# matthewygf/Tiresias

Hardware: AMD Instinct MI355X
Metric: avg JCT + makespan on NSDI'19 Microsoft trace, 8×MI355X cluster (lower is better)
Workload: dtype bf16

## Files before the change

### csrc/bindings/ops.cpp

```cpp
#include <array>
#include <ATen/ATen.h>
#include <c10/hip/HIPStream.h>
#include <torch/library.h>

#include <functional>
#include <map>
#include <mutex>
#include <sstream>
#include <tuple>
#include <vector>

#include "tam/kernels.h"
#include "tam/launch.h"
#include "tam/gemm8p.h"

using at::Tensor;
using c10::optional;

namespace {

hipStream_t cur_stream(const Tensor& t) {
  return c10::hip::getCurrentHIPStream(t.device().index()).stream();
}

// ... 831 lines not shown
void maxpool_backward_op(const Tensor& dy, const Tensor& idx, const Tensor& dx, int64_t R, int64_t S,
                         int64_t st, int64_t pad) {
  check_bf16(dy, "dy"); check_bf16(dx, "dx");
  tam::maxpool_backward(bp(dy), idx.data_ptr<uint8_t>(), bpm(dx), (int)dx.size(0), (int)dx.size(1),
                        (int)dx.size(2), (int)dx.size(3), (int)dy.size(1), (int)dy.size(2), (int)R,
                        (int)S, (int)st, (int)pad, cur_stream(dy));
}
void avgpool_forward_op(const Tensor& x, const Tensor& y) {
  check_bf16(x, "x"); check_bf16(y, "y"); check_contig(x, "x");
  tam::avgpool_forward(bp(x), bpm(y), (int)x.size(0), (int)(x.size(1) * x.size(2)), (int)x.size(3),
                       cur_stream(x));
}
void avgpool_backward_op(const Tensor& dy, const Tensor& dx) {
  check_bf16(dy, "dy"); check_bf16(dx, "dx"); check_contig(dx, "dx");
  tam::avgpool_backward(bp(dy), bpm(dx), (int)dx.size(0), (int)(dx.size(1) * dx.size(2)),
                        (int)dx.size(3), cur_stream(dy));
}

void softmax_xent_op(const Tensor& logits, const Tensor& labels, const optional<Tensor>& dlogits,
                     const Tensor& loss_rows, double smoothing, double grad_scale,
                     int64_t ignore_index, int64_t tm_b) {
  check_bf16(logits, "logits"); check_contig(logits, "logits");
  TORCH_CHECK(labels.scalar_type() == at::kLong && labels.is_cuda() && labels.is_contiguous(),
              "tam.xent: labels contiguous int64 GPU");
  check_f32(loss_rows, "loss_rows");
  const int64_t V = logits.size(-1), rows = logits.numel() / V;
  TORCH_CHECK(labels.numel() == rows && loss_rows.numel() == rows, "tam.xent: row count");
  TORCH_CHECK(tm_b <= 0 || rows % tm_b == 0, "tam.xent: tm_b must divide the rows");
  tam::softmax_xent(bp(logits), labels.data_ptr<int64_t>(), opt_ptr<tam::bf16_t>(dlogits),
                    loss_rows.data_ptr<float>(), rows, (int)V, (float)smoothing, (float)grad_scale,
                    ignore_index, cur_stream(logits), tm_b);
}

void embedding_forward_op(const Tensor& table, const Tensor& ids, const Tensor& out, double scale, int64_t tm_b,
                          const optional<Tensor>& pos) {
  check_bf16(table, "table"); check_bf16(out, "out"); check_contig(table, "table");
  TORCH_CHECK(ids.scalar_type() == at::kLong && ids.is_contiguous(), "tam.embedding: ids");
  const int64_t D = table.size(1);
  TORCH_CHECK(D % 8 == 0, "tam.embedding: D % 8");
  TORCH_CHECK(out.numel() == ids.numel() * D, "tam.embedding: out size");
  TORCH_CHECK(tm_b <= 0 || ids.numel() % tm_b == 0, "tam.embedding: tm_b must divide the ids");
  const tam::bf16_t* pp = nullptr;
  int64_t prow = 0;
  if (pos.has_value() && pos->defined()) {
    check_bf16(*pos, "pos"); check_contig(*pos, "pos");
    TORCH_CHECK(pos->dim() == 2 && pos->size(1) == D, "tam.embedding: pos must be [S][D]");
    prow = pos->size(0);
    TORCH_CHECK(prow > 0 && (tm_b > 0 ? ids.numel() / tm_b == prow : ids.numel() % prow == 0),
                "tam.embedding: pos rows must equal the sequence length");
    pp = bp(*pos);
  }
  tam::embedding_forward(bp(table), ids.data_ptr<int64_t>(), bpm(out), ids.numel(), (int)D,
                         (float)scale, cur_stream(table), table.size(0), tm_b, pp, prow);
}
void embedding_backward_op(const Tensor& dout, const Tensor& ids, const Tensor& gtable, double scale, int64_t tm_b) {
  check_bf16(dout, "dout"); check_f32(gtable, "gtable"); check_contig(dout, "dout");
  TORCH_CHECK(ids.scalar_type() == at::kLong && ids.is_contiguous() && gtable.dim() == 2 &&
                  dout.numel() == ids.numel() * gtable.size(1), "tam.embedding_backward: shapes");
  TORCH_CHECK(tm_b <= 0 || ids.numel() % tm_b == 0, "tam.embedding_backward: tm_b must divide the ids");
  tam::embedding_backward(bp(dout), ids.data_ptr<int64_t>(), gtable.data_ptr<float>(), ids.numel(),
                          (int)gtable.size(1), (float)scale, cur_stream(dout), gtable.size(0), tm_b);
}

void conv_dma_policy_op(int64_t p) { tam::conv_dma_policy((int)p); }
void conv_halo_policy_op(int64_t p) { tam::conv_halo_policy((int)p); }
void colsum_policy_op(int64_t p) { tam::colsum_policy((int)p); }
void attn_short_policy_op(int64_t p) { tam::attn_short_policy((int)p); }
void conv_wgrad_c64_policy_op(int64_t p) { tam::conv_wgrad_c64_policy((int)p); }
void conv_wgrad_order_op(int64_t p) { tam::conv_wgrad_order((int)p); }
void conv_stem_policy_op(int64_t p) { tam::conv_stem_policy((int)p); }
void conv_wgrad_slab_policy_op(int64_t p) { tam::conv_wgrad_slab_policy((int)p); }
void conv_wgrad_force_op(int64_t bm, int64_t bn, int64_t splits, int64_t noatomic) {
  tam::conv_wgrad_force((int)bm, (int)bn, (int)splits, (int)noatomic);
}
int g_dma_policy = 1;
TAM_KNOB(g_dma_policy)
void gemm_dma_policy_op(int64_t p, int64_t cfg) {
  g_dma_policy = (int)p;
  tam::gemm_dma_policy(p == 2 ? 1 : 0, (int)cfg);
}

void gemm8p_policy_op(int64_t mode, int64_t tile) { tam::gemm8p_policy((int)mode, (int)tile); }
void gemm_pw_policy_op(int64_t on) { tam::gemm_pw_policy((int)on); }

std::string policy_names_op() {
  std::string out;
  for (const auto& k : tam::knob_registry()) {
    if (!out.empty()) out += ",";
    out += k.name;
  }
  return out;
}
std::vector<int64_t> policy_state_op() {
  std::vector<int64_t> v;
  for (const auto& k : tam::knob_registry()) v.push_back(*k.p);
  return v;
}
void policy_load_op(std::vector<int64_t> v) {
  auto& reg = tam::knob_registry();
  TORCH_CHECK(v.size() == reg.size(), "policy_load: ", v.size(), " values for ", reg.size(), " knobs");
  for (size_t i = 0; i < reg.size(); ++i) *reg[i].p = (int)v[i];
}
void gemm8p_group_op(int64_t g) { tam::gemm8p_group((int)g); }
void gemm8p_slab_force_op(int64_t sp) { tam::gemm8p_slab_force((int)sp); }
void gemm8p_sk_force_op(int64_t on) { g_sk_force = on != 0; }
void conv_split_policy_op(int64_t p) { tam::conv_split_policy((int)p); }
void optim_grid_op(int64_t b) { tam::optim_grid((int)b); }
void optim_variant_op(int64_t v) { tam::optim_variant((int)v); }
void gemm_skinny_policy_op(int64_t on, int64_t sp, int64_t nst) {
  tam::gemm_skinny_policy((int)on, (int)sp, (int)nst);
}

void gemm_force_op(int64_t cfg, int64_t splits) {
  tam::gemm_force((int)cfg, (int)splits);
  g_forced = cfg >= 0 || splits >= 1;
}

void colsum_op(const Tensor& x, const Tensor& out) {
  check_bf16(x, "x"); check_f32(out, "out"); check_contig(x, "x");
  const int64_t C = x.size(-1);
  Tensor ws = at::empty({C % 8 == 0 ? (int64_t)tam::COLSUM_MAX_BLOCKS * C : 1},
                        x.options().dtype(at::kFloat));
  tam::colsum(bp(x), out.data_ptr<float>(), ws.data_ptr<float>(), x.numel() / C, (int)C,
              cur_stream(x));
}
void relu_backward_op(const Tensor& dy, const Tensor& y, const Tensor& dx) {
  check_bf16(dy, "dy"); check_bf16(y, "y"); check_bf16(dx, "dx");
  tam::relu_backward(bp(dy), bp(y), bpm(dx), dy.numel(), cur_stream(dy));
}
void sum_scale_op(const Tensor& x, const Tensor& out, double scale) {
  check_f32(x, "x"); check_f32(out, "out"); check_contig(x, "x");
  TORCH_CHECK(out.numel() >= 1, "tam.sum_scale: out");
  tam::sum_scale(x.data_ptr<float>(), x.numel(), out.data_ptr<float>(), (float)scale, cur_stream(x));
}
static std::pair<int64_t, int64_t> row_view(const Tensor& t, const char* what) {
  TORCH_CHECK(t.is_cuda() && t.scalar_type() == at::kBFloat16 && t.dim() >= 1 && t.stride(-1) == 1,
              "tam.rows_sum: ", what, " must be a bf16 CUDA tensor with unit last stride");
  const int64_t C = t.size(-1);
  int64_t ld = t.dim() >= 2 ? t.stride(-2) : C;
  for (int64_t d = t.dim() - 2; d >= 1; --d)
    TORCH_CHECK(t.size(d) == 1 || t.size(d - 1) == 1 || t.stride(d - 1) == t.stride(d) * t.size(d),
                "tam.rows_sum: ", what, " leading dims do not collapse to one row pitch");
  TORCH_CHECK(C % 8 == 0 && ld % 8 == 0 && (((uintptr_t)t.data_ptr()) & 15) == 0,
              "tam.rows_sum: ", what, " needs C % 8 == 0 and 16-B aligned rows");
  return {C, ld};
}
void rows_sum_op(at::TensorList outs, at::TensorList ins, at::IntArrayRef n_in) {
  TORCH_CHECK(!outs.empty() && outs.size() <= 4 && outs.size() == n_in.size(), "tam.rows_sum: 1-4 jobs");
  const int64_t R = outs[0].numel() / outs[0].size(-1);
  tam::RowJobs jb{};
  size_t q = 0;
  for (size_t j = 0; j < outs.size(); ++j) {
    auto [C, ld] = row_view(outs[j], "out");
    TORCH_CHECK(outs[j].numel() / C == R, "tam.rows_sum: every job needs the same row count");
    TORCH_CHECK(n_in[j] >= 1 && n_in[j] <= 4 && q + n_in[j] <= ins.size(), "tam.rows_sum: n_in");
    tam::RowJob& r = jb.job[j];
    r.out = bpm(outs[j]); r.ld_out = ld; r.C = (int)C; r.n_in = (int)n_in[j];
    for (int k = 0; k < r.n_in; ++k, ++q) {
      auto [Ci, ldi] = row_view(ins[q], "in");
      TORCH_CHECK(Ci == C && ins[q].numel() / Ci == R, "tam.rows_sum: input shape");
      r.in[k] = bp(ins[q]); r.ld_in[k] = ldi;
    }
  }
  TORCH_CHECK(q == ins.size(), "tam.rows_sum: unused inputs");
  tam::rows_sum(jb, (int)outs.size(), R, cur_stream(outs[0]));
}
// ... 206 lines not shown
                               act.data_ptr<float>(), (int)T, (int)B, (int)Hd, reverse ? 1 : 0,
                               (unsigned*)sp, cur_stream(gx), pl_opts(job_err, grids, rsv, zeroed));
}
bool lstm_seq_bwd_op(const Tensor& act, const Tensor& cs, const Tensor& dH, const Tensor& w_hh,
                     const Tensor& dG, bool reverse, const Tensor& sync, const optional<Tensor>& job_err,
                     int64_t grids, int64_t rsv, bool zeroed) {
  check_f32(act, "act"); check_f32(cs, "cs"); check_bf16(w_hh, "w_hh");
  TORCH_CHECK(dH.is_cuda() && (dH.scalar_type() == at::kFloat || dH.scalar_type() == at::kBFloat16),
              "tam.lstm_seq_backward: dH must be an f32 or bf16 CUDA tensor");
  const int dh_bf16 = dH.scalar_type() == at::kBFloat16 ? 1 : 0;
  check_bf16(dG, "dG");
  TORCH_CHECK(cs.dim() == 3 && cs.is_contiguous(), "tam.lstm_seq_backward: cs [T][B][Hd]");
  const int64_t T = cs.size(0), B = cs.size(1), Hd = cs.size(2);
  check_sync(sync, B);
  TORCH_CHECK(w_hh.is_contiguous() && w_hh.size(0) == 4 * Hd && w_hh.size(1) == Hd,
              "tam.lstm_seq_backward: w_hh [4Hd][Hd]");
  TORCH_CHECK(dH.dim() == 3 && dH.size(0) == T && dH.size(1) == B && dH.size(2) == Hd && dH.stride(2) == 1 &&
                  dH.stride(1) >= Hd && dH.stride(0) == B * dH.stride(1),
              "tam.lstm_seq_backward: dH [T][B][Hd] with unit column stride and uniform row pitch");
  TORCH_CHECK(act.is_contiguous() && act.numel() == T * B * 5 * Hd && dG.is_contiguous() &&
                  dG.numel() == T * B * 4 * Hd,
              "tam.lstm_seq_backward: act / dG shapes");
  int* sp = sync.data_ptr<int>();
  return tam::lstm_seq_backward(act.data_ptr<float>(), cs.data_ptr<float>(), (const float*)dH.data_ptr(),
                                bp(w_hh), bpm(dG), (int)T, (int)B, (int)Hd, reverse ? 1 : 0, (unsigned*)sp,
                                dh_bf16, (int)dH.stride(1), cur_stream(act), pl_opts(job_err, grids, rsv, zeroed));
}

void lstm_seq_policy_op(int64_t ch) { tam::lstm_seq_policy((int)ch); }
void lstm_seq_shards_op(int64_t ns) { tam::lstm_seq_shards((int)ns); }
void lstm_seq_residency_op(int64_t grids, int64_t rsv) { tam::lstm_seq_residency((int)grids, (int)rsv); }
int64_t lstm_persist_timeouts_op(bool reset) { return tam::lstm_persist_timeouts(reset); }
void lstm_seq_spin_limit_op(int64_t polls) { tam::lstm_seq_spin_limit(polls); }

void lstm_bwd_op(const Tensor& act, const optional<Tensor>& c_prev, const optional<Tensor>& dh,
                 const optional<Tensor>& dc_next, const optional<Tensor>& dgates,
                 const optional<Tensor>& dc_prev, const optional<Tensor>& dgates_bf16) {
  check_f32(act, "act");
  const int B = (int)act.size(0), Hd = (int)(act.size(1) / 5);
  tam::lstm_cell_backward(act.data_ptr<float>(), opt_ptr<const float>(c_prev), nullptr,
                          opt_ptr<const float>(dh), opt_ptr<const float>(dc_next),
                          opt_ptr<float>(dgates), opt_ptr<float>(dc_prev),
                          opt_ptr<tam::bf16_t>(dgates_bf16), B, Hd, c10::hip::getCurrentHIPStream(act.device().index()).stream());
}

}

TORCH_LIBRARY(tam, m) {
  m.def("gemm(Tensor a, bool a_kmajor, Tensor b, bool b_kmajor, Tensor(a!) c, int mode, Tensor? bias, bool relu, Tensor? mask, float alpha, bool allow_split, Tensor(b!)? colsum=None) -> ()", &gemm_op);
  m.def("conv_fwd(Tensor x, Tensor w, Tensor(a!) y, int stride, int pad, int dil, Tensor? bias, bool relu, Tensor(b!)? stats=None) -> int", &conv_fwd_op);
  m.def("conv_dgrad(Tensor dy, Tensor w, Tensor(a!) wt, Tensor(b!) dx, int stride, int pad, int dil, Tensor? mask) -> ()", &conv_dgrad_op);
  m.def("conv_weight_t_batch(Tensor[] w, Tensor(a!)[] wt) -> ()", &conv_weight_t_batch_op);
  m.def("gemm_wgrad_grouped(Tensor[] dy, Tensor[] x, Tensor(a!)[] dw, Tensor(b!)[] db, int[]? modes=None) -> ()", &gemm_wgrad_grouped_op);
  m.def("gemm_wgrad_grouped_ok(int M, int N, int K) -> bool", &gemm_wgrad_grouped_ok_op);
  m.def("gemm_grouped_tile(int tile) -> ()", &gemm_grouped_tile_op);
  m.def("conv_dgrad_pre(Tensor dy, Tensor w, Tensor wt, Tensor(a!) dx, int stride, int pad, int dil, Tensor? mask, Tensor(b!)? stats=None, Tensor? bnx=None, Tensor? bnmean=None, Tensor? bnrstd=None) -> int", &conv_dgrad_pre_op);
  m.def("conv_wgrad(Tensor dy, Tensor x, Tensor(a!) dw, int stride, int pad, int dil, int mode, Tensor(b!)? dbias=None, bool patch=True) -> ()", &conv_wgrad_op);
  m.def("conv_wgrad_deferred(Tensor dy, Tensor x, Tensor(a!) dw, int stride, int pad, int dil, int mode, Tensor(b!)? dbias, bool patch) -> (Tensor, int)", &conv_wgrad_deferred_op);
  m.def("wgrad_slab_reduce_many(Tensor[] slabs, int[] sp, Tensor(a!)[] dw, int[] mode) -> ()", &wgrad_slab_reduce_many_op);
  m.def("bn_forward(Tensor x, Tensor? res, Tensor(a!) y, Tensor gamma, Tensor beta, Tensor(b!)? run_mean, Tensor(c!)? run_var, Tensor(d!) save_mean, Tensor(e!) save_rstd, float eps, float momentum, bool relu, Tensor(f!)? sums=None, bool sums_ready=False, Tensor(g!)? ymask=None) -> ()", &bn_forward_op);
  m.def("bn_backward(Tensor dy, Tensor? y, Tensor x, Tensor mean, Tensor rstd, Tensor gamma, Tensor(a!) dx, Tensor(b!)? dres, Tensor(c!)? dgamma, Tensor(d!)? dbeta, bool relu, Tensor? addend=None, Tensor(e!)? sums=None, bool sums_ready=False, Tensor? ymask=None) -> ()", &bn_backward_op);
  m.def("ln_forward(Tensor x, Tensor g, Tensor b, Tensor(a!) y, Tensor(b!) mean, Tensor(c!) rstd, float eps, Tensor? addend=None, Tensor(d!)? sum_out=None, Tensor? drop_rec=None, int drop_site=0, int drop_thr=0, float drop_scale=1.0) -> ()", &ln_forward_op);
  m.def("ln_backward(Tensor dy, Tensor x, Tensor g, Tensor mean, Tensor rstd, Tensor(a!) dx, Tensor(b!) dg, Tensor(c!) db, Tensor? addend=None, Tensor(d!)? dr=None, Tensor? drop_rec=None, int drop_site=0, int drop_thr=0, float drop_scale=1.0) -> ()", &ln_backward_op);
  m.def("ln_backward_split(Tensor dy, Tensor x, Tensor g, Tensor mean, Tensor rstd, Tensor(a!) dx, Tensor(b!) ws, Tensor? addend=None, Tensor(c!)? dr=None, Tensor? drop_rec=None, int drop_site=0, int drop_thr=0, float drop_scale=1.0) -> int", &ln_backward_split_op);
  m.def("dropout_apply(Tensor x, Tensor(a!) y, Tensor rec, int site, int thr, float scale) -> ()", &dropout_apply_op);
  m.def("dropout_advance(Tensor(a!) rec) -> ()", &dropout_advance_op);
  m.def("col_reduce_acc(Tensor part, int nblk, int W, Tensor(a!) out0, Tensor(b!) out1, int split) -> ()", &col_reduce_acc_op);
  m.def("col_reduce_acc_batch(Tensor[] parts, int[] nblk, Tensor(a!)[] out0, Tensor(b!)[] out1) -> ()", &col_reduce_acc_batch_op);
  m.def("maxpool_forward(Tensor x, Tensor(a!) y, Tensor(b!) idx, int R, int S, int stride, int pad) -> ()", &maxpool_forward_op);
  m.def("maxpool_backward(Tensor dy, Tensor idx, Tensor(a!) dx, int R, int S, int stride, int pad) -> ()", &maxpool_backward_op);
  m.def("maxpool_k3s2_policy(int policy) -> ()", &maxpool_k3s2_policy_op);
  m.def("avgpool_forward(Tensor x, Tensor(a!) y) -> ()", &avgpool_forward_op);
  m.def("avgpool_backward(Tensor dy, Tensor(a!) dx) -> ()", &avgpool_backward_op);
  m.def("softmax_xent(Tensor logits, Tensor labels, Tensor(a!)? dlogits, Tensor(b!) loss_rows, float smoothing, float grad_scale, int ignore_index, int tm_b=0) -> ()", &softmax_xent_op);
  m.def("embedding_forward(Tensor table, Tensor ids, Tensor(a!) out, float scale, int tm_b=0, Tensor? pos=None) -> ()", &embedding_forward_op);
  m.def("embedding_backward(Tensor dout, Tensor ids, Tensor(a!) gtable, float scale, int tm_b=0) -> ()", &embedding_backward_op);
  m.def("sum_scale(Tensor x, Tensor(a!) out, float scale) -> ()", &sum_scale_op);
  m.def("rows_sum(Tensor[] outs, Tensor[] ins, int[] n_in) -> ()", &rows_sum_op);
  m.def("zero_(Tensor(a!) t) -> ()", &zero_op);
  m.def("colsum(Tensor x, Tensor(a!) out) -> ()", &colsum_op);
  m.def("gemm_force(int cfg, int splits) -> ()", &gemm_force_op);
  m.def("gemm8p_policy(int mode, int tile) -> ()", &gemm8p_policy_op);
  m.def("gemm_pw_policy(int on) -> ()", &gemm_pw_policy_op);
  m.def("policy_names() -> str", &policy_names_op);
  m.def("policy_state() -> int[]", &policy_state_op);
  m.def("policy_load(int[] v) -> ()", &policy_load_op);
  m.def("gemm8p_group(int g) -> ()", &gemm8p_group_op);
  m.def("gemm8p_slab_force(int sp) -> ()", &gemm8p_slab_force_op);
  m.def("gemm_skinny_policy(int on, int force_splits, int nst) -> ()", &gemm_skinny_policy_op);
  m.def("gemm8p_sk_force(int on) -> ()", &gemm8p_sk_force_op);
  m.def("conv_split_policy(int p) -> ()", &conv_split_policy_op);
  m.def("optim_variant(int v) -> ()", &optim_variant_op);
  m.def("optim_grid(int blocks) -> ()", &optim_grid_op);
  m.def("gemm_lib_policy(int policy) -> ()", &gemm_lib_policy_op);
  m.def("conv_dma_policy(int policy) -> ()", &conv_dma_policy_op);
  m.def("conv_wgrad_force(int bm, int bn, int splits, int noatomic=0) -> ()", &conv_wgrad_force_op);
  m.def("conv_wgrad_c64_policy(int policy) -> ()", &conv_wgrad_c64_policy_op);
  m.def("conv_wgrad_order(int flat) -> ()", &conv_wgrad_order_op);
  m.def("conv_stem_policy(int policy) -> ()", &conv_stem_policy_op);
  m.def("conv_wgrad_slab_policy(int policy) -> ()", &conv_wgrad_slab_policy_op);
  m.def("conv_halo_policy(int policy) -> ()", &conv_halo_policy_op);
  m.def("colsum_policy(int policy) -> ()", &colsum_policy_op);
  m.def("attn_short_policy(int policy) -> ()", &attn_short_policy_op);
  m.def("gemm_dma_policy(int policy, int cfg) -> ()", &gemm_dma_policy_op);
  m.def("gemm_routes() -> str", &gemm_routes_op);
  m.def("relu_backward(Tensor dy, Tensor y, Tensor(a!) dx) -> ()", &relu_backward_op);
  m.def("add(Tensor a, Tensor b, Tensor(a!) y) -> ()", &add_op);
  m.def("cast_f32_bf16(Tensor x, Tensor(a!) y) -> ()", &cast_op);
  m.def("sgd_step(Tensor(a!) w, Tensor(b!) g, Tensor(c!) mom, Tensor(d!) wb, float lr, float momentum, float wd, float gscale, bool nesterov, bool zero_grad, Tensor? guard=None, int zero_from=0, int wd_until=-1, Tensor? clip=None) -> ()", &sgd_op);
  m.def("adam_step(Tensor(a!) w, Tensor(b!) g, Tensor(c!) m, Tensor(d!) v, Tensor(e!) wb, float lr, float b1, float b2, float eps, float wd, int step, float gscale, bool zero_grad, Tensor? guard=None, int zero_from=0, int wd_until=-1, Tensor? clip=None) -> ()", &adam_op);
  m.def("grad_sumsq(Tensor g, Tensor(a!) partials) -> ()", &grad_sumsq_op);
  m.def("grad_clip_finalize(Tensor partials, float max_norm, float gscale, Tensor(a!) clip) -> ()", &grad_clip_finalize_op);
  m.def("grad_sumsq_blocks(int n) -> int", &grad_sumsq_blocks_op);
  m.def("lstm_guard_step(Tensor(a!) err) -> ()", &lstm_guard_step_op);
  m.def("attn_forward(Tensor q, Tensor k, Tensor v, Tensor(a!) o, Tensor(b!) lse, bool causal, float scale, Tensor? kv_len, Tensor? drop_rec=None, int drop_site=0, int drop_thr=0, float drop_scale=1.0) -> ()", &attn_forward_op);
  m.def("attn_backward(Tensor q, Tensor k, Tensor v, Tensor o, Tensor dout, Tensor lse, Tensor(a!) dq, Tensor(b!) dk, Tensor(c!) dv, Tensor(d!) dq_acc, Tensor(e!) delta, bool causal, float scale, Tensor? kv_len, Tensor? drop_rec=None, int drop_site=0, int drop_thr=0, float drop_scale=1.0) -> ()", &attn_backward_op);
  m.def("lstm_step_forward(Tensor gx, Tensor w_hh, Tensor? h_prev, Tensor? c_prev, Tensor(a!) c_out, Tensor(b!) h_out, Tensor(c!) act) -> ()", &lstm_step_fwd_op);
  m.def("lstm_seq_forward(Tensor gx, Tensor w_hh, Tensor(a!) hs, Tensor(b!) cs, Tensor(c!) act, bool reverse, Tensor(d!) sync, Tensor(e!)? job_err=None, int grids=-1, int reserved_cus=0, bool zeroed=False) -> bool", &lstm_seq_fwd_op);
  m.def("lstm_seq_backward(Tensor act, Tensor cs, Tensor dH, Tensor w_hh, Tensor(a!) dG, bool reverse, Tensor(b!) sync, Tensor(c!)? job_err=None, int grids=-1, int reserved_cus=0, bool zeroed=False) -> bool", &lstm_seq_bwd_op);
  m.def("lstm_seq_policy(int ch) -> ()", &lstm_seq_policy_op);
  m.def("lstm_seq_shards(int ns) -> ()", &lstm_seq_shards_op);
  m.def("gemm_routes_load(str text) -> int", &gemm_routes_load_op);
  m.def("lstm_seq_residency(int grids, int reserved_cus) -> ()", &lstm_seq_residency_op);
  m.def("lstm_persist_timeouts(bool reset) -> int", &lstm_persist_timeouts_op);
  m.def("lstm_seq_spin_limit(int polls) -> ()", &lstm_seq_spin_limit_op);
  m.def("lstm_cell_forward(Tensor gates, Tensor? c_prev, Tensor(a!) c_out, Tensor(b!) h_out, Tensor(c!)? h_f32, Tensor(d!) act) -> ()", &lstm_fwd_op);
  m.def("lstm_cell_backward(Tensor act, Tensor? c_prev, Tensor? dh, Tensor? dc_next, Tensor(a!)? dgates, Tensor(b!)? dc_prev, Tensor(c!)? dgates_bf16) -> ()", &lstm_bwd_op);
}
```

### csrc/include/tam/launch.h

```cpp
#pragma once
#include <hip/hip_runtime.h>
#include "tam/igemm.h"

namespace tam {

void gemm_igemm(const bf16_t* A, long lda, bool a_kmajor, const bf16_t* B, long ldb, bool b_kmajor, int M,
                int N, int K, const Epi& ep, hipStream_t s);
void gemm(const bf16_t* A, long lda, bool a_kmajor, const bf16_t* B, long ldb, bool b_kmajor,
          int M, int N, int K, Epi ep, bool allow_split, hipStream_t s);
void gemm_select(const bf16_t* A, long lda, bool a_kmajor, const bf16_t* B, long ldb, bool b_kmajor,
                 int M, int N, int K, Epi ep, bool allow_split, hipStream_t s, int path);
void gemm_force(int cfg, int splits);
void gemm_dma_policy(int policy, int cfg);
void gemm8p_policy(int mode, int tile);
bool gemm_pw(const bf16_t* A, long lda, const bf16_t* B, long ldb, bf16_t* C, long ldc, long M, int N, int K,
             const bf16_t* mask, long ldm, double* stats, int relu, hipStream_t s);
bool gemm_pw_ok(long M, int N, int K, long lda, long ldb, long ldc);
void gemm_pw_policy(int on);
void gemm8p_group(int g);
int gemm8p_policy_mode();

struct GGProblem {
  const bf16_t* A;
  const bf16_t* B;
  float* C;
  float* bias;
  int M, N, K, lda, ldb;
  int mode = 1;
};
void gemm_wgrad_grouped(const GGProblem* probs, int n, hipStream_t s);
void wgrad_slab_reduce_many(const float* const* ws, const int* sp, const long* mn, float* const* dw,
                            const int* mode, int n, hipStream_t s);
bool gemm_wgrad_grouped_ok(int M, int N, int K, long lda, long ldb);
void gemm_grouped_tile(int t);

void gemm_slab_reduce(const float* ws, int sp, int M, int N, const Epi& ep, hipStream_t s);

bool gemm_skinny_ok(bool ak, bool bk, int M, int N, int K, long lda, long ldb);
int gemm_skinny_splits(int M, int N, int K);
void gemm_skinny(const bf16_t* A, long lda, const bf16_t* B, long ldb, bool bk, int M, int N, int K,
                 const Epi& ep, int sp, float* ws, hipStream_t s);
void gemm_skinny_policy(int on, int force_splits, int nst);

int conv_fwd(const bf16_t* x, const bf16_t* w, const ConvGeom& g, Epi ep, hipStream_t s, float* ws = nullptr,
             long ws_floats = 0);
long conv_fwd_split_ws(const ConvGeom& g);
bool conv_stem_fwd(const bf16_t* x, const bf16_t* w, const ConvGeom& g, const Epi& ep, hipStream_t s);
void conv_stem_policy(int p);
long conv_stem_wgrad_ws(const ConvGeom& g);
bool conv_stem_wgrad(const bf16_t* dy, const bf16_t* x, const ConvGeom& g, float* dw, int mode, float* ws,
                     long ws_floats, hipStream_t s);
long conv_dgrad_split_ws(const ConvGeom& g);
void conv_split_policy(int p);
int conv_dgrad(const bf16_t* dy, const bf16_t* w, const bf16_t* wt, const ConvGeom& g, Epi ep,
               hipStream_t s, float* ws = nullptr, long ws_floats = 0);
int conv_wgrad(const bf16_t* dy, const bf16_t* x, const ConvGeom& g, Epi ep, hipStream_t s,
               float* dbias = nullptr, bool allow_patch = true, float* ws = nullptr, long ws_floats = 0,
               int* slab_defer = nullptr);
long conv_wgrad_split_ws(const ConvGeom& g);
void conv_wgrad_slab_policy(int p);
void conv_weight_t(const bf16_t* w, bf16_t* wt, const ConvGeom& g, hipStream_t s);
void conv_dma_policy(int p);
void conv_wgrad_force(int bm, int bn, int splits, int noatomic = 0);
void conv_wgrad_order(int flat);
void conv_wgrad_c64_policy(int p);
void conv_halo_policy(int p);
bool gemm_select_big_p8(bool ak, bool bk, int M, int N, int K, long lda, long ldb);

}
```

### csrc/kernels/conv.hip

```cpp
#include <cstdlib>

#include "tam/launch.h"
#include "tam/tiles.h"
#include "tam/conv_dma.h"
#include "tam/kernels.h"

namespace tam {

static int g_conv_dma = 1;
TAM_KNOB(g_conv_dma)
void conv_dma_policy(int p) { g_conv_dma = p; }
static int g_conv_split = 1;
TAM_KNOB(g_conv_split)
void conv_split_policy(int p) { g_conv_split = p; }
static int g_conv_halo = [] {
  const char* e = getenv("TAM_CONV_HALO");
  return e ? atoi(e) : 1;
}();
TAM_KNOB(g_conv_halo)
void conv_halo_policy(int p) { g_conv_halo = p; }
static ::tam::KnobReg g_wgrad_force_knobs_[4] = {{"g_wgrad_force0", &g_wgrad_force[0]}, {"g_wgrad_force1", &g_wgrad_force[1]},
                                                  {"g_wgrad_force2", &g_wgrad_force[2]}, {"g_wgrad_force3", &g_wgrad_force[3]}};
void conv_wgrad_force(int bm, int bn, int splits, int noatomic) {
  g_wgrad_force[0] = bm; g_wgrad_force[1] = bn; g_wgrad_force[2] = splits; g_wgrad_force[3] = noatomic;
}

template <int BM, int BN>
static void fwd_tile(const bf16_t* x, const bf16_t* w, const ConvGeom& g, const Epi& ep, int sp,
                     hipStream_t s) {
  const int M = g.N * g.P * g.Q, Kd = g.R * g.S * g.C;
  LdConvFwdA<BM> la{x, g, M, Kd};
  la.with_divs();
  LdKMajor<BN> lb{w, Kd, g.K, Kd};
  launch_igemm<BM, BN>(la, lb, M, g.K, Kd, ep, sp, s);
}

static bool is_pointwise(const ConvGeom& g) {
  return g.R == 1 && g.S == 1 && g.stride == 1 && g.pad == 0;
}

long conv_fwd_split_ws(const ConvGeom& g) {
  if (!g_conv_dma || g.dil != 1 || !g_conv_split) return 0;
  return conv_dma_split_ws(cd_fwd_args(nullptr, nullptr, g), g_conv_dma >= 2 ? g_conv_dma - 1 : 0);
}
long conv_dgrad_split_ws(const ConvGeom& g) {
  if (!g_conv_dma || g.dil != 1 || g.stride != 1 || !g_conv_split) return 0;
  CDArgs a = cd_dgrad_args(nullptr, nullptr, g, 0, 0);
  const int force = g_conv_dma >= 2 ? g_conv_dma - 1 : (g.C == 64 && a.M >= (1L << 20) ? 1 : 0);
  return conv_dma_split_ws(a, force);
}


int conv_fwd(const bf16_t* x, const bf16_t* w, const ConvGeom& g, Epi ep, hipStream_t s, float* ws,
             long ws_floats) {
  const int M = g.N * g.P * g.Q, Kd = g.R * g.S * g.C;
  if (conv_stem_fwd(x, w, g, ep, s)) return ep.stats ? 1 : 0;
  if (is_pointwise(g) && !ep.c_f32 && ep.mode == 0 && !ep.bias && !ep.mask && ep.alpha == 1.f &&
      gemm_pw(x, g.C, w, g.C, (bf16_t*)ep.c, ep.ldc, M, g.K, g.C, nullptr, 0, ep.stats, ep.relu, s))
    return ep.stats ? 1 : 0;
  if (g_conv_dma && g.dil == 1) {
    CDArgs a = cd_fwd_args(x, w, g);
    if (g_conv_halo && launch_conv_halo(a, ep, s)) return ep.stats ? 1 : 0;
    const int force = g_conv_dma >= 2 ? g_conv_dma - 1 : 0;
    const int bm = launch_conv_dma(a, ep, s, force, ws, ws_floats);
    if (bm) return ep.stats ? 1 : 0;
  }
  if (is_pointwise(g)) {
    ep.stats = nullptr;
    gemm(x, g.C, true, w, g.C, true, M, g.K, g.C, ep, false, s);
    return 0;
  }
  ep.stats = nullptr;
  TileChoice t = choose_tiles(M, g.K, Kd, false);
  switch (t.cfg) {
    case 0: fwd_tile<128, 128>(x, w, g, ep, 1, s); break;
    case 1: fwd_tile<128, 64>(x, w, g, ep, 1, s); break;
    case 2: fwd_tile<64, 128>(x, w, g, ep, 1, s); break;
    default: fwd_tile<64, 64>(x, w, g, ep, 1, s); break;
  }
  return 0;
}

template <int BM, int BN>
static void dgrad_tile(const bf16_t* dy, const bf16_t* wt, const ConvGeom& g, const Epi& ep,
                       hipStream_t s) {
  const int M = g.N * g.H * g.W, Kd = g.R * g.S * g.K;
  LdConvDgradA<BM> la{dy, g, M, Kd};
  la.with_divs();
  LdKMajor<BN> lb{wt, Kd, g.C, Kd};
  launch_igemm<BM, BN>(la, lb, M, g.C, Kd, ep, 1, s);
}

int conv_dgrad(const bf16_t* dy, const bf16_t* w, const bf16_t* wt, const ConvGeom& g, Epi ep,
               hipStream_t s, float* ws, long ws_floats) {
  const int M = g.N * g.H * g.W, Kd = g.R * g.S * g.K;
  if (wt && g_conv_dma && g.dil == 1 && g.stride == 1) {
    CDArgs a = cd_dgrad_args(dy, wt, g, 0, 0);
    if (g_conv_halo && launch_conv_halo(a, ep, s)) return ep.stats ? 1 : 0;
    static const long dg64_min_m = [] {
      const char* e = getenv("TAM_DGRAD64_MIN_M");
      return e ? atol(e) : (1L << 20);
    }();
    const int force = g_conv_dma >= 2 ? g_conv_dma - 1 : (g.C == 64 && a.M >= dg64_min_m ? 1 : 0);
    const int bm = launch_conv_dma(a, ep, s, force, ws, ws_floats);
    if (bm) return ep.stats ? 1 : 0;
  }
  ep.stats = nullptr;
  ep.bnx = nullptr;
  if (wt && g_conv_dma && g.dil == 1 && g.stride > 1 && g.K % 64 == 0 && g.C % 64 == 0 &&
      ep.mode == 0 && !ep.c_f32 && g.stride * g.stride <= 4) {
    CDArgs cls[4];
    bool ok = true, empty = false;
    for (int ph = 0, i = 0; ph < g.stride; ++ph)
      for (int pw = 0; pw < g.stride; ++pw, ++i) {
        cls[i] = cd_dgrad_args(dy, wt, g, ph, pw);
        if (cls[i].ntaps == 0) empty = true;
        else ok = ok && conv_dma_pick_bn(cls[i].M, cls[i].Ng, cls[i].Kd, 1) != 0;
      }
    if (ok) {
      if (empty) zero_async(ep.c, (size_t)M * g.C * sizeof(bf16_t), s);
      CDArgs live[4];
      int n = 0;
      for (int i = 0; i < g.stride * g.stride; ++i)
        if (cls[i].ntaps) live[n++] = cls[i];
      if (g_conv_dma == 3 || !launch_conv_dma_multi(live, n, ep, s))
        for (int i = 0; i < n; ++i) launch_conv_dma(live[i], ep, s, g_conv_dma == 3 ? 2 : 1);
      return 0;
    }
  }
  if (is_pointwise(g)) {
    if (wt && !ep.c_f32 && ep.mode == 0 && !ep.bias && ep.alpha == 1.f && !ep.relu &&
        gemm_pw(dy, g.K, wt, g.K, (bf16_t*)ep.c, ep.ldc, M, g.C, g.K, ep.mask, ep.ldm, nullptr, 0, s))
      return 0;
    gemm(dy, g.K, true, w, g.C, false, M, g.C, g.K, ep, false, s);
    return 0;
  }
  TileChoice t = choose_tiles(M, g.C, Kd, false);
  switch (t.cfg) {
    case 0: dgrad_tile<128, 128>(dy, wt, g, ep, s); break;
    case 1: dgrad_tile<128, 64>(dy, wt, g, ep, s); break;
    case 2: dgrad_tile<64, 128>(dy, wt, g, ep, s); break;
    default: dgrad_tile<64, 64>(dy, wt, g, ep, s); break;
  }
  return 0;
}

template <int BM, int BN>
static void wgrad_tile(const bf16_t* dy, const bf16_t* x, const ConvGeom& g, const Epi& ep, int sp,
                       hipStream_t s) {
  const int Mred = g.N * g.P * g.Q, Nc = g.R * g.S * g.C;
  LdMNMajor<BM> la{dy, g.K, g.K, Mred};
  LdConvWgradB<BN> lb{x, g, Mred, Nc};
  lb.with_divs();
  launch_igemm<BM, BN>(la, lb, g.K, Nc, Mred, ep, sp, s);
}

static int g_wgrad_c64 = 1;
TAM_KNOB(g_wgrad_c64) TAM_KNOB(g_wgrad_slab)
void conv_wgrad_c64_policy(int p) { g_wgrad_c64 = p; }
void conv_wgrad_order(int flat) { g_wgrad_flat = flat; }
void conv_wgrad_slab_policy(int p) { g_wgrad_slab = p; }
long conv_wgrad_split_ws(const ConvGeom& g) {
  const long stem = conv_stem_wgrad_ws(g);
  if (stem > 0) return stem;
  if (!g_conv_dma || (is_pointwise(g) && (long)g.N * g.P * g.Q < 100352 && g_conv_dma < 2)) return 0;
  return wgrad_dma_slab_floats(g, g_conv_dma >= 2);
}

int conv_wgrad(const bf16_t* dy, const bf16_t* x, const ConvGeom& g, Epi ep, hipStream_t s, float* dbias,
               bool allow_patch, float* ws, long ws_floats, int* slab_defer) {
  if (slab_defer) *slab_defer = 0;
  const int Mred = g.N * g.P * g.Q, Nc = g.R * g.S * g.C;
  if (!dbias && ep.c_f32 && ep.ldc == Nc && ep.mode <= 1 &&
      conv_stem_wgrad(dy, x, g, (float*)ep.c, ep.mode, ws, ws_floats, s))
    return 0;
  if (g_conv_dma && g_wgrad_c64 && (allow_patch || g_wgrad_c64 >= 2) && (g.K == 64 || g_wgrad_c64 >= 2) &&
      ep.c_f32 && ep.ldc == Nc && ep.mode <= 1 &&
      launch_conv_wgrad_c64(dy, x, (float*)ep.c, g, ep.mode, g_wgrad_c64 >= 2 ? g_wgrad_c64 : 0, s,
// ... 112 lines not shown
```

### csrc/kernels/gemm_pw.hip

```cpp
#include "tam/launch.h"
#include "tam/kernels.h"

namespace tam {

struct PwArgs {
  const bf16_t* A;
  long lda;
  const bf16_t* B;
  long ldb;
  bf16_t* C;
  long ldc;
  long M;
  const bf16_t* mask;
  long ldm;
  double* stats;
  int relu;
};

template <int K, int N>
__global__ void __launch_bounds__(256, 2) gemm_pw_kernel(PwArgs a) {
  constexpr int KT = K / 32, NT = N / 16;
  constexpr int BLD = K + 8;
  constexpr int SLD = N + 8;
  constexpr int CPR = N / 8;
// ... 49 lines not shown
    __builtin_amdgcn_sched_barrier(0);
    f32x4_t acc[NT];
#pragma unroll
    for (int j = 0; j < NT; ++j) acc[j] = f32x4_t{0.f, 0.f, 0.f, 0.f};
#pragma unroll
    for (int ks = 0; ks < KT; ++ks)
#pragma unroll
      for (int j = 0; j < NT; ++j) {
        const s16x8_t bf = *(const s16x8_t*)(Bs + (16 * j + r16) * BLD + 32 * ks + koff);
        acc[j] = __builtin_amdgcn_mfma_f32_16x16x32_bf16(__builtin_bit_cast(bf16x8_t, cur.af[ks]),
                                                         __builtin_bit_cast(bf16x8_t, bf), acc[j], 0, 0, 0);
      }
    bf16_t* sl = slab[w];
#pragma unroll
    for (int j = 0; j < NT; ++j)
#pragma unroll
      for (int r = 0; r < 4; ++r) {
        float v = acc[j][r];
        if (a.relu) v = fmaxf(v, 0.f);
        sl[(4 * (lane >> 4) + r) * SLD + 16 * j + r16] = f2bf(v);
      }
    asm volatile("s_waitcnt lgkmcnt(0)" ::: "memory");
#pragma unroll
    for (int u = 0; u < S; ++u) {
      const int lr = u * RPU + lane / CPR;
      const long m = mt * 64 + 16 * w + lr;
      const long ms = m < a.M ? m : a.M - 1;
      uint4 v = *(const uint4*)(sl + lr * SLD + ch * 8);
      if (a.mask) {
        uint4 mk;
        if constexpr (MPRE) mk = cur.mk[u];
        else mk = *(const uint4*)(a.mask + ms * a.ldm + ch * 8);
        const uint32_t* mw = (const uint32_t*)&mk;
        uint32_t* vw = (uint32_t*)&v;
#pragma unroll
        for (int e = 0; e < 4; ++e) {
          const uint32_t m2 = mw[e];
          const bool lo = (m2 & 0x8000u) == 0 && (m2 & 0x7fffu) != 0;
          const bool hi = (m2 & 0x80000000u) == 0 && (m2 & 0x7fff0000u) != 0;
          vw[e] &= (lo ? 0x0000ffffu : 0u) | (hi ? 0xffff0000u : 0u);
        }
      }
      *(uint4*)(a.C + ms * a.ldc + ch * 8) = v;
      if (stats) {
        const float inr = m < a.M ? 1.f : 0.f;
        const uint32_t* vw = (const uint32_t*)&v;
#pragma unroll
        for (int e = 0; e < 4; ++e) {
          const float lo = __uint_as_float(vw[e] << 16) * inr, hi = __uint_as_float(vw[e] & 0xffff0000u) * inr;
          ssum[2 * e] += lo; ssq[2 * e] += lo * lo;
          ssum[2 * e + 1] += hi; ssq[2 * e + 1] += hi * hi;
        }
      }
    }
  };
  Regs r0, r1;
  long mt = blockIdx.x;
  if (mt < ntiles) issue(mt, r0);
  for (; mt < ntiles; mt += 2 * (long)gridDim.x) {
    tile(mt, r0, r1);
    if (mt + gridDim.x < ntiles) tile(mt + gridDim.x, r1, r0);
  }
  if (!stats) return;
#pragma unroll
  for (int o = CPR; o < 64; o <<= 1)
#pragma unroll
    for (int e = 0; e < 8; ++e) {
      ssum[e] += __shfl_xor(ssum[e], o, 64);
      ssq[e] += __shfl_xor(ssq[e], o, 64);
    }
  if (lane < CPR) {
#pragma unroll
    for (int e = 0; e < 8; ++e) {
      red[w][lane * 8 + e] = ssum[e];
      red[w][N + lane * 8 + e] = ssq[e];
    }
  }
  __syncthreads();
  double* sh = a.stats + (long)(blockIdx.x % BN_SHARDS) * 2 * N;
  for (int e = tid; e < 2 * N; e += 256)
    unsafeAtomicAdd(sh + e, (double)(red[0][e] + red[1][e] + red[2][e] + red[3][e]));
}

static int g_conv_pw = [] {
  const char* e = getenv("TAM_CONV_PW");
  return e ? atoi(e) : 1;
}();
TAM_KNOB(g_conv_pw)
void gemm_pw_policy(int on) { g_conv_pw = on; }

bool gemm_pw_ok(long M, int N, int K, long lda, long ldb, long ldc) {
  if (!g_conv_pw || M < 65536) return false;
  const bool kn = (K == 64 || K == 128 || K == 256) && (N == 64 || N == 128 || N == 256) && K * N <= 16384;
  return kn && lda % 8 == 0 && ldb % 8 == 0 && ldc % 8 == 0;
}

template <int K, int N>
static void pw_launch(const PwArgs& a, hipStream_t s) {
  static const long resident = [] {
    int dev = 0, per_cu = 1;
    hipDeviceProp_t prop;
    TAM_HIP_CHECK(hipGetDevice(&dev));
    TAM_HIP_CHECK(hipGetDeviceProperties(&prop, dev));
    TAM_HIP_CHECK(hipOccupancyMaxActiveBlocksPerMultiprocessor(&per_cu, gemm_pw_kernel<K, N>, 256, 0));
    return (long)(per_cu < 1 ? 1 : per_cu) * prop.multiProcessorCount;
  }();
  const long ntiles = (a.M + 63) / 64;
  const long blocks = ntiles < resident ? ntiles : resident;
  hipLaunchKernelGGL((gemm_pw_kernel<K, N>), dim3((unsigned)blocks), dim3(256), 0, s, a);
}

bool gemm_pw(const bf16_t* A, long lda, const bf16_t* B, long ldb, bf16_t* C, long ldc, long M, int N, int K,
             const bf16_t* mask, long ldm, double* stats, int relu, hipStream_t s) {
  if (!gemm_pw_ok(M, N, K, lda, ldb, ldc)) return false;
  if (mask && ldm % 8 != 0) return false;
  const PwArgs a{A, lda, B, ldb, C, ldc, M, mask, ldm, stats, relu};
  switch (K * 1000 + N) {
    case 64064: pw_launch<64, 64>(a, s); return true;
    case 64128: pw_launch<64, 128>(a, s); return true;
    case 64256: pw_launch<64, 256>(a, s); return true;
    case 128064: pw_launch<128, 64>(a, s); return true;
    case 128128: pw_launch<128, 128>(a, s); return true;
    case 256064: pw_launch<256, 64>(a, s); return true;
    default: return false;
  }
}

}
```

Baseline: 0.1374.

## Add wide pointwise GEMM kernel and route pointwise conv dgrad through it

Adds a 512-thread pointwise GEMM kernel for wider N/K shapes (128x256, 128x512, 256x512). It streams weight chunks through double-buffered shared memory, keeps activation rows in registers, and stages outputs through a per-wave shared slab with an optional mask and BN-stat reduction. Pointwise conv dgrad calls now try this kernel first when the epilogue is plain. The goal is to replace the general conv/GEMM path for these large 1x1 layers with a specialised persistent kernel. A torch binding and a max_blocks cap are added for testing. Fixed minimum-M thresholds per shape gate the new kernel, and it risks being slower than the tuned generic path.

Measured after the change: 0.1366, median of 5. About the same (-0.6%).

```diff
diff --git a/csrc/bindings/ops.cpp b/csrc/bindings/ops.cpp
--- a/csrc/bindings/ops.cpp
+++ b/csrc/bindings/ops.cpp
@@ -937,6 +937,31 @@
 
 void gemm8p_policy_op(int64_t mode, int64_t tile) { tam::gemm8p_policy((int)mode, (int)tile); }
 void gemm_pw_policy_op(int64_t on) { tam::gemm_pw_policy((int)on); }
+bool gemm_pw_op(const Tensor& a, const Tensor& b, const Tensor& c, const optional<Tensor>& mask,
+                const optional<Tensor>& stats, bool relu, int64_t max_blocks) {
+  check_bf16(a, "a"); check_bf16(b, "b"); check_bf16(c, "c");
+  TORCH_CHECK(a.dim() == 2 && b.dim() == 2 && c.dim() == 2 && a.size(1) == b.size(1) && c.size(0) == a.size(0) &&
+                  c.size(1) == b.size(0) && a.size(0) > 0,
+              "tam.gemm_pw: shapes a [M,K], b [N,K], c [M,N] expected");
+  auto rows = [](const Tensor& t) { return t.size(1) == 1 || t.stride(1) == 1; };
+  TORCH_CHECK(rows(a) && rows(b) && rows(c), "tam.gemm_pw: operand rows must be contiguous");
+  const tam::bf16_t* mk = nullptr;
+  long ldm = 0;
+  if (mask.has_value() && mask->defined()) {
+    check_bf16(*mask, "mask");
+    TORCH_CHECK(mask->dim() == 2 && mask->sizes() == c.sizes() && rows(*mask), "tam.gemm_pw: mask [M,N] expected");
+    mk = bp(*mask); ldm = mask->stride(0);
+  }
+  double* st = nullptr;
+  if (stats.has_value() && stats->defined()) {
+    TORCH_CHECK(stats->is_cuda() && stats->scalar_type() == at::kDouble && stats->is_contiguous() &&
+                    stats->numel() == tam::BN_SHARDS * 2 * c.size(1),
+                "tam.gemm_pw: stats must be fp64 [BN_SHARDS * 2N]");
+    st = stats->data_ptr<double>();
+  }
+  return tam::gemm_pw(bp(a), a.stride(0), bp(b), b.stride(0), bpm(c), c.stride(0), a.size(0), (int)b.size(0),
+                      (int)a.size(1), mk, ldm, st, relu ? 1 : 0, cur_stream(a), (int)max_blocks);
+}
 
 std::string policy_names_op() {
   std::string out;
@@ -1309,6 +1334,7 @@
   m.def("gemm_force(int cfg, int splits) -> ()", &gemm_force_op);
   m.def("gemm8p_policy(int mode, int tile) -> ()", &gemm8p_policy_op);
   m.def("gemm_pw_policy(int on) -> ()", &gemm_pw_policy_op);
+  m.def("gemm_pw(Tensor a, Tensor b, Tensor(a!) c, Tensor? mask, Tensor(b!)? stats, bool relu, int max_blocks=0) -> bool", &gemm_pw_op);
   m.def("policy_names() -> str", &policy_names_op);
   m.def("policy_state() -> int[]", &policy_state_op);
   m.def("policy_load(int[] v) -> ()", &policy_load_op);
diff --git a/csrc/include/tam/launch.h b/csrc/include/tam/launch.h
--- a/csrc/include/tam/launch.h
+++ b/csrc/include/tam/launch.h
@@ -14,8 +14,9 @@
 void gemm_dma_policy(int policy, int cfg);
 void gemm8p_policy(int mode, int tile);
 bool gemm_pw(const bf16_t* A, long lda, const bf16_t* B, long ldb, bf16_t* C, long ldc, long M, int N, int K,
-             const bf16_t* mask, long ldm, double* stats, int relu, hipStream_t s);
+             const bf16_t* mask, long ldm, double* stats, int relu, hipStream_t s, int max_blocks = 0);
 bool gemm_pw_ok(long M, int N, int K, long lda, long ldb, long ldc);
+bool gemm_pw_is_wide(int N, int K);
 void gemm_pw_policy(int on);
 void gemm8p_group(int g);
 int gemm8p_policy_mode();
diff --git a/csrc/kernels/conv.hip b/csrc/kernels/conv.hip
--- a/csrc/kernels/conv.hip
+++ b/csrc/kernels/conv.hip
@@ -94,6 +94,10 @@
 int conv_dgrad(const bf16_t* dy, const bf16_t* w, const bf16_t* wt, const ConvGeom& g, Epi ep,
                hipStream_t s, float* ws, long ws_floats) {
   const int M = g.N * g.H * g.W, Kd = g.R * g.S * g.K;
+  if (is_pointwise(g) && wt && gemm_pw_is_wide(g.C, g.K) && !ep.stats && !ep.bnx && !ep.c_f32 && ep.mode == 0 &&
+      !ep.bias && ep.alpha == 1.f && !ep.relu &&
+      gemm_pw(dy, g.K, wt, g.K, (bf16_t*)ep.c, ep.ldc, M, g.C, g.K, ep.mask, ep.ldm, nullptr, 0, s))
+    return 0;
   if (wt && g_conv_dma && g.dil == 1 && g.stride == 1) {
     CDArgs a = cd_dgrad_args(dy, wt, g, 0, 0);
     if (g_conv_halo && launch_conv_halo(a, ep, s)) return ep.stats ? 1 : 0;
diff --git a/csrc/kernels/gemm_pw.hip b/csrc/kernels/gemm_pw.hip
--- a/csrc/kernels/gemm_pw.hip
+++ b/csrc/kernels/gemm_pw.hip
@@ -155,6 +155,142 @@
     unsafeAtomicAdd(sh + e, (double)(red[0][e] + red[1][e] + red[2][e] + red[3][e]));
 }
 
+
+template <int K, int N>
+__global__ void __launch_bounds__(512, 4) gemm_pw_wide_kernel(PwArgs a) {
+  constexpr int NC = 64, KC = 128;
+  constexpr int KT = K / 32, NCH = N / NC, KCH = K / KC;
+  constexpr int NU = KCH % 2 == 0 ? 1 : 2;
+  constexpr int BLD = KC + 8;
+  constexpr int SLD = NC + 8;
+  constexpr int CPR = NC / 8;
+  constexpr int RPU = 64 / CPR;
+  constexpr int S = 16 / RPU;
+  static_assert(K % KC == 0 && N % NC == 0 && NCH % NU == 0, "gemm_pw_wide shape");
+  __shared__ __attribute__((aligned(16))) bf16_t Bs[2][NC * BLD];
+  __shared__ __attribute__((aligned(16))) bf16_t slab[8][16 * SLD];
+  __shared__ float red[2 * N];
+  const int tid = threadIdx.x, lane = tid & 63, w = tid >> 6;
+  const int r16 = lane & 15, koff = 8 * (lane >> 4);
+  const bool stats = a.stats != nullptr;
+
+  const int bn0 = tid >> 4, bc = (tid & 15) * 8;
+  auto load_b = [&](int nc, int kc, uint4 (&b)[2]) {
+    const bf16_t* src = a.B + (long)(nc * NC + bn0) * a.ldb + kc * KC + bc;
+    b[0] = *(const uint4*)src;
+    b[1] = *(const uint4*)(src + 32 * a.ldb);
+  };
+  auto store_b = [&](int buf, const uint4 (&b)[2]) {
+    *(uint4*)(Bs[buf] + bn0 * BLD + bc) = b[0];
+    *(uint4*)(Bs[buf] + (bn0 + 32) * BLD + bc) = b[1];
+  };
+  const long ntiles = (a.M + 127) / 128;
+  if ((long)blockIdx.x >= ntiles) return;
+  {
+    uint4 b[2];
+    load_b(0, 0, b);
+    for (int e = tid; e < 2 * N; e += 512) red[e] = 0.f;
+    store_b(0, b);
+  }
+  __syncthreads();
+
+  const int ch = lane % CPR;
+  bf16_t* sl = slab[w];
+  for (long mt = blockIdx.x; mt < ntiles; mt += gridDim.x) {
+    s16x8_t af[KT];
+    {
+      long m = mt * 128 + 16 * w + r16;
+      m = m < a.M ? m : a.M - 1;
+#pragma unroll
+      for (int ks = 0; ks < KT; ++ks) af[ks] = *(const s16x8_t*)(a.A + m * a.lda + 32 * ks + koff);
+    }
+    float inr[4];
+#pragma unroll
+    for (int r = 0; r < 4; ++r) inr[r] = mt * 128 + 16 * w + 4 * (lane >> 4) + r < a.M ? 1.f : 0.f;
+    f32x4_t acc[NC / 16];
+#pragma unroll 1
+    for (int nc0 = 0; nc0 < NCH; nc0 += NU)
+#pragma unroll
+    for (int uu = 0; uu < NU * KCH; ++uu) {
+      const int nc = nc0 + uu / KCH, kc = uu % KCH, buf = uu & 1;
+      uint4 nb[2];
+      load_b(kc + 1 < KCH ? nc : (nc + 1 < NCH ? nc + 1 : 0), kc + 1 < KCH ? kc + 1 : 0, nb);
+      uint4 mk[S];
+      if (kc == KCH - 1 && a.mask) {
+#pragma unroll
+        for (int t = 0; t < S; ++t) {
+          long m = mt * 128 + 16 * w + t * RPU + lane / CPR;
+          m = m < a.M ? m : a.M - 1;
+          mk[t] = *(const uint4*)(a.mask + m * a.ldm + nc * NC + ch * 8);
+        }
+      }
+      if (kc == 0) {
+#pragma unroll
+        for (int j = 0; j < NC / 16; ++j) acc[j] = f32x4_t{0.f, 0.f, 0.f, 0.f};
+      }
+#pragma unroll
+      for (int ks = 0; ks < KC / 32; ++ks)
+#pragma unroll
+        for (int j = 0; j < NC / 16; ++j) {
+          const s16x8_t bf = *(const s16x8_t*)(Bs[buf] + (16 * j + r16) * BLD + 32 * ks + koff);
+          acc[j] = __builtin_amdgcn_mfma_f32_16x16x32_bf16(__builtin_bit_cast(bf16x8_t, af[kc * (KC / 32) + ks]),
+                                                           __builtin_bit_cast(bf16x8_t, bf), acc[j], 0, 0, 0);
+        }
+      store_b(buf ^ 1, nb);
+      if (kc == KCH - 1) {
+#pragma unroll
+        for (int j = 0; j < NC / 16; ++j) {
+          float cs = 0.f, cq = 0.f;
+#pragma unroll
+          for (int r = 0; r < 4; ++r) {
+            float v = acc[j][r];
+            if (a.relu) v = fmaxf(v, 0.f);
+            const bf16_t h = f2bf(v);
+            sl[(4 * (lane >> 4) + r) * SLD + 16 * j + r16] = h;
+            if (stats) {
+              const float vr = bf2f(h) * inr[r];
+              cs += vr; cq += vr * vr;
+            }
+          }
+          if (stats) {
+            cs += __shfl_xor(cs, 16, 64); cq += __shfl_xor(cq, 16, 64);
+            cs += __shfl_xor(cs, 32, 64); cq += __shfl_xor(cq, 32, 64);
+            if (lane < 16) {
+              __hip_atomic_fetch_add(&red[nc * NC + 16 * j + lane], cs, __ATOMIC_RELAXED, __HIP_MEMORY_SCOPE_WORKGROUP);
+              __hip_atomic_fetch_add(&red[N + nc * NC + 16 * j + lane], cq, __ATOMIC_RELAXED,
+                                     __HIP_MEMORY_SCOPE_WORKGROUP);
+            }
+          }
+        }
+        asm volatile("s_waitcnt lgkmcnt(0)" ::: "memory");
+#pragma unroll
+        for (int t = 0; t < S; ++t) {
+          const int lr = t * RPU + lane / CPR;
+          const long m = mt * 128 + 16 * w + lr;
+          const long ms = m < a.M ? m : a.M - 1;
+          uint4 v = *(const uint4*)(sl + lr * SLD + ch * 8);
+          if (a.mask) {
+            const uint32_t* mw = (const uint32_t*)&mk[t];
+            uint32_t* vw = (uint32_t*)&v;
+#pragma unroll
+            for (int e = 0; e < 4; ++e) {
+              const uint32_t m2 = mw[e];
+              const bool lo = (m2 & 0x8000u) == 0 && (m2 & 0x7fffu) != 0;
+              const bool hi = (m2 & 0x80000000u) == 0 && (m2 & 0x7fff0000u) != 0;
+              vw[e] &= (lo ? 0x0000ffffu : 0u) | (hi ? 0xffff0000u : 0u);
+            }
+          }
+          *(uint4*)(a.C + ms * a.ldc + nc * NC + ch * 8) = v;
+        }
+      }
+      __syncthreads();
+    }
+  }
+  if (!stats) return;
+  double* sh = a.stats + (long)(blockIdx.x % BN_SHARDS) * 2 * N;
+  for (int e = tid; e < 2 * N; e += 512) unsafeAtomicAdd(sh + e, (double)red[e]);
+}
+
 static int g_conv_pw = [] {
   const char* e = getenv("TAM_CONV_PW");
   return e ? atoi(e) : 1;
@@ -162,39 +298,77 @@
 TAM_KNOB(g_conv_pw)
 void gemm_pw_policy(int on) { g_conv_pw = on; }
 
+static bool pw_narrow_shape(int N, int K) {
+  return (K == 64 || K == 128 || K == 256) && (N == 64 || N == 128 || N == 256) && K * N <= 16384;
+}
+
+static long pw_wide_min_m(int N, int K) {
+  switch (K * 10000 + N) {
+    case 1280256: return 200704;
+    case 1280512: return 50176;
+    case 2560512: return 50176;
+    default: return 0;
+  }
+}
+
+bool gemm_pw_is_wide(int N, int K) { return pw_wide_min_m(N, K) != 0; }
+
 bool gemm_pw_ok(long M, int N, int K, long lda, long ldb, long ldc) {
-  if (!g_conv_pw || M < 65536) return false;
-  const bool kn = (K == 64 || K == 128 || K == 256) && (N == 64 || N == 128 || N == 256) && K * N <= 16384;
-  return kn && lda % 8 == 0 && ldb % 8 == 0 && ldc % 8 == 0;
+  if (!g_conv_pw || M < 1) return false;
+  if (lda % 8 != 0 || ldb % 8 != 0 || ldc % 8 != 0 || lda < K || ldb < K || ldc < N) return false;
+  if (pw_narrow_shape(N, K)) return g_conv_pw >= 2 || M >= 65536;
+  const long min_m = pw_wide_min_m(N, K);
+  return min_m != 0 && (g_conv_pw >= 2 || M >= min_m);
+}
+
+template <typename Kern>
+static long pw_resident(Kern kern, int threads) {
+  int dev = 0, per_cu = 1;
+  hipDeviceProp_t prop;
+  TAM_HIP_CHECK(hipGetDevice(&dev));
+  TAM_HIP_CHECK(hipGetDeviceProperties(&prop, dev));
+  TAM_HIP_CHECK(hipOccupancyMaxActiveBlocksPerMultiprocessor(&per_cu, kern, threads, 0));
+  return (long)(per_cu < 1 ? 1 : per_cu) * prop.multiProcessorCount;
 }
 
 template <int K, int N>
-static void pw_launch(const PwArgs& a, hipStream_t s) {
-  static const long resident = [] {
-    int dev = 0, per_cu = 1;
-    hipDeviceProp_t prop;
-    TAM_HIP_CHECK(hipGetDevice(&dev));
-    TAM_HIP_CHECK(hipGetDeviceProperties(&prop, dev));
-    TAM_HIP_CHECK(hipOccupancyMaxActiveBlocksPerMultiprocessor(&per_cu, gemm_pw_kernel<K, N>, 256, 0));
-    return (long)(per_cu < 1 ? 1 : per_cu) * prop.multiProcessorCount;
-  }();
+static void pw_launch(const PwArgs& a, int max_blocks, hipStream_t s) {
+  static const long resident = pw_resident(gemm_pw_kernel<K, N>, 256);
   const long ntiles = (a.M + 63) / 64;
-  const long blocks = ntiles < resident ? ntiles : resident;
+  long blocks = ntiles < resident ? ntiles : resident;
+  if (max_blocks > 0 && blocks > max_blocks) blocks = max_blocks;
   hipLaunchKernelGGL((gemm_pw_kernel<K, N>), dim3((unsigned)blocks), dim3(256), 0, s, a);
 }
 
+template <int K, int N>
+static void pw_wide_launch(const PwArgs& a, int max_blocks, hipStream_t s) {
+  static const long resident = pw_resident(gemm_pw_wide_kernel<K, N>, 512);
+  const long ntiles = (a.M + 127) / 128;
+  long blocks = ntiles < resident ? ntiles : resident;
+  if (max_blocks > 0 && blocks > max_blocks) blocks = max_blocks;
+  hipLaunchKernelGGL((gemm_pw_wide_kernel<K, N>), dim3((unsigned)blocks), dim3(512), 0, s, a);
+}
+
 bool gemm_pw(const bf16_t* A, long lda, const bf16_t* B, long ldb, bf16_t* C, long ldc, long M, int N, int K,
-             const bf16_t* mask, long ldm, double* stats, int relu, hipStream_t s) {
+             const bf16_t* mask, long ldm, double* stats, int relu, hipStream_t s, int max_blocks) {
   if (!gemm_pw_ok(M, N, K, lda, ldb, ldc)) return false;
-  if (mask && ldm % 8 != 0) return false;
+  if (mask && (ldm % 8 != 0 || ldm < N)) return false;
   const PwArgs a{A, lda, B, ldb, C, ldc, M, mask, ldm, stats, relu};
-  switch (K * 1000 + N) {
-    case 64064: pw_launch<64, 64>(a, s); return true;
-    case 64128: pw_launch<64, 128>(a, s); return true;
-    case 64256: pw_launch<64, 256>(a, s); return true;
-    case 128064: pw_launch<128, 64>(a, s); return true;
-    case 128128: pw_launch<128, 128>(a, s); return true;
-    case 256064: pw_launch<256, 64>(a, s); return true;
+  switch (K * 10000 + N) {
+    case 640064: pw_launch<64, 64>(a, max_blocks, s); return true;
+    case 640128: pw_launch<64, 128>(a, max_blocks, s); return true;
+    case 640256: pw_launch<64, 256>(a, max_blocks, s); return true;
+    case 1280064: pw_launch<128, 64>(a, max_blocks, s); return true;
+    case 1280128: pw_launch<128, 128>(a, max_blocks, s); return true;
+    case 2560064: pw_launch<256, 64>(a, max_blocks, s); return true;
+    default: break;
+  }
+  if (mask && stats) return false;
+  if (stats && g_conv_pw < 2) return false;
+  switch (K * 10000 + N) {
+    case 1280256: pw_wide_launch<128, 256>(a, max_blocks, s); return true;
+    case 1280512: pw_wide_launch<128, 512>(a, max_blocks, s); return true;
+    case 2560512: pw_wide_launch<256, 512>(a, max_blocks, s); return true;
     default: return false;
   }
 }
```
